# ISAE-PNX/SaDVIO

Measured on AMD Instinct MI355X. Metric: BA iterations/sec (ms/solve in ms_per_solve), 20-KF/8k-landmark window, higher is better.
Workload: dtype f64; 1 GPU; synthetic 20 KF x 8000 landmarks x 40000 reprojection factors (pixel), GN 10 iters (LM step attempts, early exits disabled); windows_per_gpu=1, parallelism=single window, n_kf=20, n_lmk=8000, n_obs=40000, reduced_dim=114

## Files before the change

sadvio_amd/csrc/ba_handle.h:

```cpp
#pragma once
#include <hip/hip_runtime.h>
#include <dlfcn.h>

#include <algorithm>
#include <chrono>
#include <cmath>
#include <cstdio>
#include <cstdlib>
#include <cstring>
#include <map>
#include <string>
#include <vector>

#include "../../include/sadvio_ba.h"
#include "kernels.h"
#include "layout_plan.h"
#include "dense_chol.h"
#include "marg_kernels.h"
#include "lm_kernels.h"
#include "long_kernels.h"
#include "viinit_kernels.h"
#include "nofov_kernels.h"

using namespace sadvio;
// ... 191 lines not shown
    ~CovBatchScratch() { if (pinned) (void)hipHostFree(pinned); }
};

struct RelScratch {
    DevBuf<int> pairs, kf_ptr, kf_lmk, n_shared, status;
    DevBuf<double> inf, Ak, Tab;
    std::vector<int> h_pairs, h_ptr, h_lmk, h_last;
    int csr_win = -1;
    int n_kf_lmk = 0;
};

struct EnvCfg {
    int debug = 0;
    int lm = -1, pf_wg = -1;
    int tile_rounds = 0, lm_subs = 0, band_c = 0;
    int cov_batch_lds = 1, cov_batch_scratch_mb = 1024;
    int cov_band = -1;
    int cov_sqrt = -1;
    int cov_cross_stage = -1;
    int long_min = 0;
    int long_min_env = 0;
    double jacobi_tol = 1e-14;
    bool marg_pivoted = false, marg_unpivoted = false, pchol_strict = false, no_lpt = false, no_pre = false, no_fork = false, no_bcr = false, imu_items = false, contig_tiles = false, c16_old_tail = false;
    void read() {
        auto on = [](const char* k) { return getenv(k) != nullptr; };
        auto num = [](const char* k, int unset) { const char* e = getenv(k); return e ? atoi(e) : unset; };
        debug = num("SADVIO_DEBUG", 0); lm = num("SADVIO_LM", -1); pf_wg = num("SADVIO_PF_WG", -1);
        tile_rounds = num("SADVIO_TILE_ROUNDS", 0); lm_subs = num("SADVIO_LM_SUBS", 0); band_c = num("SADVIO_BAND_C", 0);
        cov_batch_lds = num("SADVIO_COV_BATCH_LDS", 1); cov_batch_scratch_mb = num("SADVIO_COV_BATCH_SCRATCH_MB", 1024);
        cov_band = num("SADVIO_COV_BAND", -1); cov_sqrt = num("SADVIO_COV_SQRT", -1);
        cov_cross_stage = num("SADVIO_COV_CROSS_STAGE", -1);
        long_min_env = num("SADVIO_LONG_MIN", 0);
        if (long_min_env < 2 || long_min_env > MAX_LMK_OBS + 1) long_min_env = 0;
        if (const char* e = getenv("SADVIO_JACOBI_TOL")) jacobi_tol = atof(e);
        marg_pivoted = on("SADVIO_MARG_PIVOTED"); marg_unpivoted = on("SADVIO_MARG_UNPIVOTED"); pchol_strict = on("SADVIO_PCHOL_STRICT");
        no_lpt = on("SADVIO_NO_LPT"); no_pre = on("SADVIO_NO_PRE"); no_fork = on("SADVIO_NO_FORK");
        no_bcr = on("SADVIO_NO_BCR");
        contig_tiles = on("SADVIO_CONTIG_TILES");
        c16_old_tail = on("SADVIO_C16_OLD_TAIL");
        imu_items = on("SADVIO_IMU_ITEMS");
    }
};

struct sadvio_ba_handle {
    EnvCfg env;
    sadvio_ba_config cfg{};
    LayoutPlan plan;
    int device = 0;
    hipStream_t stream = nullptr;
    std::string err;
    std::vector<PriorDev> priors;
    std::vector<std::vector<PriorDev>> priors_per_win;
    std::vector<std::vector<ImuDev>> imus_per_win;
    std::vector<ImuDev> imus;
    DevBuf<int> d_big_info;
    DevBuf<double> d_big_M;
    DevBuf<double> d_big_Lx;
    DevBuf<double> d_big_linv;
    DevBuf<double> d_coll_band;
    DevBuf<double> d_bcr;
// ... 21 lines not shown
    DevBuf<LineDev> d_lines;
    DevBuf<LineObsDev> d_lobs;
    DevBuf<double> d_xline, d_line_scratch;
    int n_line_tot = 0, n_lobs_tot = 0;
    DevBuf<SparseDev> d_sparse;
    DevBuf<int> d_sp_list;
    int n_sp_list = 0;
    size_t n_sparse_tot = 0;
    DevBuf<double> d_sp_scratch;
    DevBuf<int> d_lmk_red, d_kept_obs, d_dp_ints;
    DevBuf<double> d_dp_data;
    int last_slots = 0;
    DevBuf<WinDev> d_win;
    DevBuf<Tile> d_tiles;
    DevBuf<double> d_kf_T0, d_xp, d_xv, d_xba, d_xbg, d_kf_vel, d_kf_ba, d_kf_bg;
    DevBuf<int> d_kf_fidx;
    DevBuf<double> d_cam_K, d_cam_T, d_cam_isig;
    DevBuf<double> d_lmk_p, d_xl, d_s_lmk;
    DevBuf<unsigned char> d_lmk_const;
    DevBuf<int> d_lmk_ob, d_lmk_oe, d_obs_kf, d_obs_cam, d_tile_kf, d_tile_row, d_tile_lmk;
    DevBuf<int> d_long_rec, d_long_kf, d_long_slot;
    DevBuf<int> d_pre_lane, d_pre_kf;
    bool pre_dirty = false;
    DevBuf<int> d_rank_col; DevBuf<double> d_rank_x;
    DevBuf<unsigned char> d_obs_slot, d_obs_lslot;
    DevBuf<int> d_chunk_ob, d_chunk_lm, d_tile_perm;
    DevBuf<int> d_jac_ints;
    DevBuf<double> d_jac_dbl;
    DevBuf<double> d_lm_hg, d_lm_dt, d_lm_sacc;
    DevBuf<int> d_lm_sub;
    int hidden_eig_count = 0;
    int marg_stats[4] = {0, 0, 0, 0};
    DevBuf<double> d_ptab;
    DevBuf<double> d_obs_meas;
    DevBuf<PriorDev> d_priors;
    DevBuf<double> d_prior_lin;
    DevBuf<ImuDev> d_imus;
    DevBuf<double> d_imu_scratch;
    DevBuf<double> d_S, d_gred, d_gfull, d_hdiag, d_delta, d_s_pose;
    DevBuf<LmState> d_states;
    DevBuf<double> d_trace;
    DevBuf<long long> d_tstart;
    DevBuf<IterAcc> d_acc;
    DevBuf<FinalRec> d_final;
    FinalRec* h_final = nullptr;
    double* h_deltas = nullptr; size_t h_deltas_cap = 0; bool deltas_cached = false;
// ... 70 lines not shown
```

sadvio_amd/csrc/ba_types.h:

```cpp
#pragma once
#include <stdint.h>

namespace sadvio {

struct SolveOpts {
    int max_num_iterations;
    int jacobi_scaling;
    int max_num_consecutive_invalid_steps;
    int pad;
    double function_tolerance, gradient_tolerance, parameter_tolerance;
    double initial_radius, max_radius, min_radius;
    double min_lm_diagonal, max_lm_diagonal, min_relative_decrease;
    double huber_a;
    double max_time_ticks;
};

struct WinDev {
    int n_kf, n_cam, n_lmk, n_obs;
    int kf_base, cam_base, lmk_base, obs_base;
    int n_free_kf, dpf, Np, Npose;
    long long S_off;
    int red_off;
    int tile_begin, tile_end;
    int prior_begin, prior_end;
// ... 7 lines not shown
    int kept_begin, kept_end;
    int sp_begin, sp_end;
    int spl_begin, spl_end;
    int line_begin, line_end;
    int lobs_begin, lobs_end;
};

struct Tile {
    int w;
    int lmk0, lmk1;
    int lmk_off;
    int n_lmk;
    int G;
    int kf_off, n_kf;
    int n_free;
    int lds_mode;
    int dpf, Np;
    int red_off;
    int cam_base, n_cam;
    int first_of_window;
    int kmax;
    int win_tile0, win_ntiles;
    int ld;
    long long S_off;
    int chunk0, chunk1;
};

struct PriorDev {
    int kf;
    int pad;
    double T_prior[12];
    double inf[6];
};

struct ImuDev {
    int kf_i, kf_j;
    double dt;
    double dR[9], dv[3], dp[3];
    double J_dR_bg[9], J_dv_ba[9], J_dv_bg[9], J_dp_ba[9], J_dp_bg[9];
    double W[81];
    double sa, sg;
    int win, pad;
};
struct SparseDev {
    int type, kf, lmk0, lmk1;
    int win, kf2;
// ... 51 lines not shown
    double lin_cost, fixed_cost, gmax;
    double cand_cost, mcc, step_norm2, cand_norm2;
    double pad;
};

constexpr int BUILD_THREADS = 256;
constexpr int BUILD_WAVES = BUILD_THREADS / 64;
constexpr int MAX_TILE_KF = 24;
constexpr int MAX_TILE_FREE_KF = 20;
constexpr int MAX_GEMM_FREE_KF = 5;
constexpr int MAX_WIN_CAM = 8;
constexpr int STAGE_VALS = 18;
constexpr int MAX_LMK_OBS = 64;
constexpr int MAX_LONG_OBS = 4096;
constexpr int MAX_LONG_KF = 512;
constexpr int LONG_THREADS = 256;
constexpr int LONG_REC = 6;
constexpr int SOLVE_THREADS = 512;
constexpr int SOLVE_KFC_STRIDE = 32;
constexpr int SOLVE_KFC = 32;
constexpr int PRIOR_LIN = 28;
constexpr int PRE_KF = 8;
constexpr int PRE_MAX_TILES = 1024;
constexpr int MAX_LDS_NP = 174;
constexpr int LM_CHUNK = 12;
constexpr int LM_PASS_THREADS = 64;

constexpr int c16_blocks(int n_rows) { return (n_rows + 15) >> 4; }
constexpr int c16_size(int N) { return (c16_blocks(N + 1) * (c16_blocks(N + 1) + 1) / 2) << 8; }

}
```

sadvio_amd/csrc/chol16.h:

```cpp
#pragma once
#include <hip/hip_runtime.h>

#include <type_traits>

#include "ba_types.h"


namespace sadvio {

typedef double c16_d4 __attribute__((ext_vector_type(4)));

constexpr int C16_STEP = 64;
constexpr int C16_PUB = 4 * C16_STEP;
constexpr int C16_WT = 16 * 17;
constexpr int C16_WORK = 2 * C16_PUB + 64 + C16_WT;

__host__ __device__ constexpr int c16_tile(int I, int J) { return ((I * (I + 1)) >> 1) + J; }
__host__ __device__ constexpr int c16_index(int i, int j) { return (c16_tile(i >> 4, j >> 4) << 8) + ((j & 15) << 4) + (i & 15); }

__device__ __forceinline__ double c16_readlane(double v, int lane) {
    int lo = __double2loint(v), hi = __double2hiint(v);
    lo = __builtin_amdgcn_readlane(lo, lane);
    hi = __builtin_amdgcn_readlane(hi, lane);
    return __hiloint2double(hi, lo);
}
__device__ __forceinline__ double c16_rsqrt(double d) {
    double y = __builtin_amdgcn_rsq(d);
    const double t = d * y;
    const double e = __builtin_fma(-t, y, 1.0);
    const double p = __builtin_fma(0.375, e, 0.5);
    const double q = e * p;
    return __builtin_fma(y, q, y);
}
__device__ __forceinline__ void c16_pair16(double v, double& e, double& o) {
    const unsigned lo = __double2loint(v), hi = __double2hiint(v);
    auto a = __builtin_amdgcn_permlane16_swap(lo, lo, false, false);
    auto b = __builtin_amdgcn_permlane16_swap(hi, hi, false, false);
    e = __hiloint2double(b[0], a[0]); o = __hiloint2double(b[1], a[1]);
}
__device__ __forceinline__ void c16_pair32(double v, double& l, double& u) {
    const unsigned lo = __double2loint(v), hi = __double2hiint(v);
// ... 404 lines not shown
```

sadvio_amd/csrc/kernels.h:

```cpp
#pragma once
#include "ba_types.h"
#include "device_math.h"
#include "chol16.h"

namespace sadvio {

struct DevPtrs {
    const WinDev* win;
    const Tile* tiles;
    const double* kf_T0;
    const int* kf_fidx;
    double* xp; double* xv; double* xba; double* xbg;
    long long xp_stride, xv_stride, xl_stride;
    const double* kf_vel; const double* kf_ba; const double* kf_bg;
    const double* cam_K; const double* cam_T; const double* cam_isig;
    const double* lmk_p; double* xl; double* s_lmk;
    const unsigned char* lmk_const;
    const int* lmk_ob; const int* lmk_oe;
    const int* obs_kf; const int* obs_cam; const double* obs_meas;
    const unsigned char* obs_slot;
    const int* tile_kf;
    const int* tile_lmk;
    const int* tile_row;
    const int4* pre_lane;
// ... 34 lines not shown
    const unsigned char* obs_lslot;
    double* lm_hg;
    double* lm_dt;
    long long lm_hg_stride, lm_dt_stride;
    const int* lm_sub;
    int lm_sub_per_item;
    int lm_ksub;
    double* lm_sacc;
    const LineDev* lines;
    const LineObsDev* lobs;
    double* xline;
    double* line_scratch;
    long long xline_stride;
    long long n_xp, n_xv, n_xl;
    int n_tiles;
    int state_stride;
    int n_win;
    long long* t_start;
    double* trace;
    long long* dbg_ts;
    int debug;
    int c16_old_tail;
    SolveOpts o;
};

#ifdef SADVIO_KERNEL_TS
#define SADVIO_TS(slot_, idx_) do { if ((P.debug & 4096) && blockIdx.x == 0 && threadIdx.x == 0 && slot == (slot_)) P.dbg_ts[idx_] = wall_clock64(); } while (0)
#define SADVIO_TS_PTR(cond_) ((cond_) ? P.dbg_ts : nullptr)
constexpr int DBG_WG_MAX = 1024, DBG_WG_BASE = 128, DBG_SLOTS = DBG_WG_BASE + 4 * DBG_WG_MAX;
#define SADVIO_WG_TS(slot_, which_) do { if ((P.debug & 4096) && blockIdx.x < DBG_WG_MAX && threadIdx.x == 0 && slot == (slot_)) { \
        P.dbg_ts[DBG_WG_BASE + 4 * blockIdx.x + (which_)] = wall_clock64(); \
        if ((which_) == 0) P.dbg_ts[DBG_WG_BASE + 4 * blockIdx.x + 3] = 0; \
        if ((which_) == 0) P.dbg_ts[DBG_WG_BASE + 4 * blockIdx.x + 2] = ((long long)__builtin_amdgcn_s_getreg(20 | (31 << 11)) << 32) | (unsigned)__builtin_amdgcn_s_getreg(4 | (31 << 11)); } } while (0)
#else
#define SADVIO_TS(slot_, idx_) do { } while (0)
#define SADVIO_TS_PTR(cond_) nullptr
#define SADVIO_WG_TS(slot_, which_) do { } while (0)
constexpr int DBG_SLOTS = 128;
#endif

__device__ __forceinline__ int tri(int i, int j) { return i * (i + 1) / 2 + j; }
__device__ __forceinline__ long long s_index(int ld, int i, int j) { return ld ? (long long)i * ld + j : (long long)c16_index(i, j); }

__device__ __forceinline__ void atomic_add_f64(double* p, double v) { unsafeAtomicAdd(p, v); }

__device__ __forceinline__ void atomic_max_u64(unsigned long long* p, unsigned long long v) { atomicMax(p, v); }
// ... 331 lines not shown
    return (b + 15) & ~(size_t)15;
}

__device__ __forceinline__ int tile_landmark(const Tile& T, const int* __restrict__ tile_lmk, int i) { return T.lmk_off >= 0 ? tile_lmk[T.lmk_off + i] : T.lmk0 + i; }

__global__ __launch_bounds__(BUILD_THREADS) void k_pre_packets(const Tile* __restrict__ tiles, const int* __restrict__ lmk_ob, const int* __restrict__ lmk_oe,
                                                               const int* __restrict__ tile_kf, const int* __restrict__ tile_lmk, const int* __restrict__ kf_fidx, int4* __restrict__ pre_lane,
                                                               int2* __restrict__ pre_kf) {
    const Tile T = tiles[blockIdx.x];
    const int tid = threadIdx.x;
    if (tid < BUILD_THREADS / 8) {
        const int lane0 = tid * 8, wv = lane0 >> 6, ln = lane0 & 63;
        const int G = T.G, lpw = 64 / G, grp = ln / G, q0 = ln - grp * G, nl = T.n_lmk;
        const bool valid = wv * lpw + grp < nl;
        const int gl = nl > 0 ? tile_landmark(T, tile_lmk, valid ? wv * lpw + grp : 0) : T.lmk0;
        const int ob = nl > 0 ? lmk_ob[gl] : 0, nobs = (valid && nl > 0) ? lmk_oe[gl] - ob : 0;
        pre_lane[(long long)blockIdx.x * (BUILD_THREADS / 8) + tid] = make_int4(gl, ob, nobs | (valid ? 1 << 16 : 0), q0);
    }
    if (tid < PRE_KF) {
        int2 e = make_int2(-1, -1);
        if (tid < T.n_kf) { e.x = tile_kf[T.kf_off + tid]; e.y = kf_fidx[e.x]; }
        pre_kf[(long long)blockIdx.x * PRE_KF + tid] = e;
    }
}

template <bool COST_ONLY> __device__ __forceinline__ void pose_factor_eval(const DevPtrs& P, int slot, int idx, int ln);
template <int FACTOR, bool RARE, bool IMU>
__global__ __launch_bounds__(BUILD_THREADS, IMU ? 1 : 2) void k_build(DevPtrs P, int slot, int max_tile_kf, int strip_doubles, int Rp) {
    extern __shared__ __attribute__((aligned(16))) char smem[];
    if (IMU && (int)blockIdx.x >= P.n_tiles) {
        pose_factor_eval<false>(P, slot, (int)blockIdx.x - P.n_tiles, threadIdx.x);
        return;
    }
    const Tile T = P.tiles[blockIdx.x];
    const int tid = threadIdx.x, wv = tid >> 6, ln = tid & 63;
    int4 pl = make_int4(0, -1, 0, 0);
    int2 pk = make_int2(-1, -1);
    if (P.pre_lane) {
        pl = P.pre_lane[(long long)blockIdx.x * (BUILD_THREADS / 8) + (tid >> 3)];
        pk = P.pre_kf[(long long)blockIdx.x * PRE_KF + tid / POSE_TAB];
    }
    SADVIO_TS(3, 32);
    SADVIO_WG_TS(3, 0);
    __shared__ double s_part[BUILD_WAVES * 4];
    double* poseTab = (double*)smem;
    double* camTab = poseTab + (size_t)max_tile_kf * POSE_TAB;
// ... 337 lines not shown
                    }
                }
            }
        }
        wave_lds_fence();
    }
        }
    if (gemm_mode && wv * lpw < nl) {
        const int lr = ln & 15, lk = ln >> 4;
        const int nt16 = (Nt + 15) >> 4;
#pragma unroll
        for (int pp = 0; pp < 3; pp++) {
            const int tr = pp < 1 ? 0 : 1, tc = pp - tr;
            if (tr < nt16) {
                const int col = 16 * tc + lr;
#pragma unroll
                for (int rg = 0; rg < 4; rg++) {
                    const int row = 16 * tr + lk + 4 * rg;
                    if (row < Nt && col <= row) atomic_add_f64(&Stile[tri(row, col)], -accs[pp][rg]);
                }
            }
        }
    }
    SADVIO_TS(3, 40);
    const double c = wave_sum(cost_part), f = wave_sum(fixed_part), gm = wave_max(gmax_part);
    if (ln == 0) { s_part[wv * 4] = c; s_part[wv * 4 + 1] = f; s_part[wv * 4 + 2] = gm; }
    __syncthreads();
    if (tid == 0) {
        double cs = 0.0, fs = 0.0, gs = 0.0;
        for (int k = 0; k < BUILD_WAVES; k++) { cs += s_part[k * 4]; fs += s_part[k * 4 + 1]; gs = fmax(gs, s_part[k * 4 + 2]); }
        TileAcc* ta = P.tacc + (long long)(slot & 1) * P.n_tiles + blockIdx.x;
        ta->lin_cost = cs; ta->fixed_cost = fs; ta->gmax = gs;
    }
    SADVIO_TS(3, 41);
    if (lds_mode) {
        int* growTab = (int*)stage;
        for (int k = tid; k < T.n_kf; k += blockDim.x) {
            const int r = rowTab[k];
            if (r >= 0) {
                const int fi = P.kf_fidx[P.tile_kf[T.kf_off + k]];
#pragma unroll
                for (int i = 0; i < 6; i++) growTab[r + i] = fi * dpf + i;
            }
        }
        __syncthreads();
        if (T.ld) {
            for (int row = wv; row < Nt; row += BUILD_WAVES) {
                const long long grow = (long long)growTab[row] * T.ld;
                const double* srow = Stile + tri(row, 0);
                for (int col = ln; col <= row; col += 64) {
                    const double v = srow[col];
                    if (v != 0.0) atomic_add_f64(&Sg[grow + growTab[col]], v);
                }
            }
        } else {
            for (int col = wv; col < Nt; col += BUILD_WAVES) {
                const int gc = growTab[col];
                for (int row = col + ln; row < Nt; row += 64) {
// ... 2243 lines not shown
```

sadvio_amd/csrc/layout_driver.h:

```cpp
#pragma once
#include "ba_handle.h"

namespace {

__global__ void k_dense_prior_prepare(const double* J, double* Jt, int nf, int n) {
    const long long idx = (long long)blockIdx.x * blockDim.x + threadIdx.x;
    if (idx < (long long)nf * n) {
        const int i = (int)(idx / n), a = (int)(idx - (long long)i * n);
        Jt[(size_t)a * nf + i] = J[idx];
    }
}

__global__ void k_sym_from_lower(const double* __restrict__ A, int n, double* __restrict__ H) {
    const long long idx = (long long)blockIdx.x * blockDim.x + threadIdx.x;
    if (idx >= (long long)n * n) return;
    const int i = (int)(idx / n), j = (int)(idx - (long long)i * n);
    H[idx] = i >= j ? A[idx] : A[(size_t)j * n + i];
}

LayoutIn layout_inputs(sadvio_ba_handle* h) {
    LayoutIn in;
    in.src = &h->src; in.sparse_per_win = &h->sparse_per_win; in.dprior_per_win = &h->dprior_per_win; in.lines_per_win = &h->lines_per_win;
    in.prior_valid = h->prior.valid; in.prior_serial = h->prior.serial; in.prior_n_full = h->prior.n_full; in.prior_n = h->prior.n;
    in.world = h->world; in.has_coll = h->coll_fn != nullptr;
    in.tile_rounds = h->env.tile_rounds; in.lm = h->env.lm; in.lm_subs = h->env.lm_subs;
    in.contig_tiles = h->env.contig_tiles; in.no_lpt = h->env.no_lpt; in.no_pre = h->env.no_pre;
    in.long_min = h->env.long_min;
    return in;
}

template <typename T>
void queue_table(sadvio_ba_handle* h, DevBuf<T>& dst, const std::vector<T>& src) { h->up.add(dst.p, src.data(), src.size() * sizeof(T)); }

int layout_reduced_device(sadvio_ba_handle* h) {
    LayoutPlan& P = h->plan;
    const long long s_b = P.s_tot, nrb = P.n_rank_b;
    const int red_b = P.np_tot;
    HIP_TRY(h->d_S.alloc((size_t)std::max<long long>(P.red_total, 1)));
    h->d_gred.set_view(h->d_S.p + s_b, (size_t)red_b); h->d_gfull.set_view(h->d_gred.p + red_b, (size_t)red_b);
    h->d_hdiag.set_view(h->d_gfull.p + red_b, (size_t)red_b); h->d_rank_b.set_view(h->d_hdiag.p + red_b, (size_t)nrb);
    HIP_TRY(h->d_rank_s.alloc((size_t)nrb));
    HIP_TRY(h->d_delta.alloc((size_t)std::max(red_b, 1))); HIP_TRY(h->d_s_pose.alloc((size_t)std::max(red_b, 1)));
    HIP_TRY(hipMemsetAsync(h->d_S.p, 0, sizeof(double) * (size_t)std::max<long long>(P.red_total, 1), h->stream));
    HIP_TRY(hipMemsetAsync(h->d_rank_s.p, 0, sizeof(double) * (size_t)nrb, h->stream));
    HIP_TRY(h->d_sparse.alloc(std::max<size_t>(P.sparse.size(), 1))); HIP_TRY(h->d_sp_scratch.alloc(2 * std::max<size_t>(P.sparse.size(), 1) * SPARSE_J));
    HIP_TRY(h->d_sp_list.alloc(std::max<size_t>(P.sp_list.size(), 1)));
    h->n_sparse_tot = P.sparse.size(); h->n_sp_list = (int)P.sp_list.size();
    h->n_line_tot = (int)P.lines.size(); h->n_lobs_tot = (int)P.lobs.size();
    HIP_TRY(h->d_lines.alloc(std::max<size_t>(P.lines.size(), 1))); HIP_TRY(h->d_lobs.alloc(std::max<size_t>(P.lobs.size(), 1)));
    HIP_TRY(h->d_xline.alloc(std::max<size_t>(12 * P.lines.size(), 1))); HIP_TRY(h->d_line_scratch.alloc(std::max<size_t>(P.lobs.size(), 1) * LINE_ROW));
    HIP_TRY(h->d_tiles.alloc(P.tiles.size())); HIP_TRY(h->d_lmk_red.alloc(P.lmk_red.size())); HIP_TRY(h->d_lmk_const.alloc(P.lmk_const_red.size()));
    HIP_TRY(h->d_kept_obs.alloc(P.kept.size())); HIP_TRY(h->d_dp_ints.alloc(P.dp_ints.size())); HIP_TRY(h->d_dp_data.alloc((size_t)std::max<long long>(P.dp_total, 1)));
    queue_table(h, h->d_sparse, P.sparse); queue_table(h, h->d_sp_list, P.sp_list); queue_table(h, h->d_lines, P.lines); queue_table(h, h->d_lobs, P.lobs);
    queue_table(h, h->d_tiles, P.tiles); queue_table(h, h->d_lmk_red, P.lmk_red); queue_table(h, h->d_lmk_const, P.lmk_const_red);
    queue_table(h, h->d_kept_obs, P.kept); queue_table(h, h->d_dp_ints, P.dp_ints);
    if (!P.preps.empty()) HIP_TRY(hipMemsetAsync(h->d_dp_data.p, 0, sizeof(double) * (size_t)P.dp_total, h->stream));
    for (const DensePrep& pr : P.preps) {
        const DensePriorHost& D = h->dprior_per_win[pr.w];
        double* J = h->d_dp_data.p + pr.off;
        double* r0 = J + 2 * (size_t)pr.nf * pr.n + (size_t)pr.n * pr.n;
        if (D.resident) {
            HIP_TRY(hipMemcpyAsync(J, h->prior.J.p, sizeof(double) * (size_t)pr.nf * pr.n, hipMemcpyDeviceToDevice, h->stream));
            HIP_TRY(hipMemcpyAsync(r0, h->prior.r0.p, sizeof(double) * (size_t)pr.nf, hipMemcpyDeviceToDevice, h->stream));
        } else {
            h->up.add(J, D.J.data(), sizeof(double) * (size_t)pr.nf * pr.n);
            h->up.add(r0, D.r0.data(), sizeof(double) * (size_t)pr.nf);
        }
    }
    if (!P.preps.empty()) HIP_TRY(h->up.flush(h->stream));
    for (const DensePrep& pr : P.preps) {
        double* J = h->d_dp_data.p + pr.off;
        double* Jt = J + (size_t)pr.nf * pr.n;
        double* H = Jt + (size_t)pr.n * pr.nf;
        const long long items = (long long)pr.nf * pr.n;
        hipLaunchKernelGGL(k_dense_prior_prepare, dim3((unsigned)((items + 255) / 256)), dim3(256), 0, h->stream, J, Jt, pr.nf, pr.n);
        if (h->dprior_per_win[pr.w].resident && h->prior.hg_valid && h->prior.n == pr.n)
            hipLaunchKernelGGL(k_sym_from_lower, dim3((unsigned)(((long long)pr.n * pr.n + 255) / 256)), dim3(256), 0, h->stream, h->prior.H.p, pr.n, H);
        else
// ... 26 lines not shown
    }
    HIP_TRY(h->d_priors.alloc(h->priors.size()));
    HIP_TRY(h->d_prior_lin.alloc(2 * h->priors.size() * (size_t)PRIOR_LIN));
    if (!h->priors.empty())
        h->up.add(h->d_priors.p, h->priors.data(), h->priors.size() * sizeof(PriorDev));
    h->imus.clear();
    for (size_t w = 0; w < wins.size(); w++) {
        wins[w].d.imu_begin = (int)h->imus.size();
        for (auto& f : h->imus_per_win[w]) { h->imus.push_back(f); h->imus.back().win = (int)w; }
        wins[w].d.imu_end = (int)h->imus.size();
    }
    HIP_TRY(h->d_imus.alloc(h->imus.size()));
    HIP_TRY(h->d_imu_scratch.alloc(2 * h->imus.size() * (size_t)IMU_ROW));
    if (!h->imus.empty())
        h->up.add(h->d_imus.p, h->imus.data(), h->imus.size() * sizeof(ImuDev));
    std::vector<WinDev> wd(wins.size());
    for (size_t w = 0; w < wins.size(); w++) wd[w] = wins[w].d;
    h->up.add(h->d_win.p, wd.data(), wd.size() * sizeof(WinDev));
    HIP_TRY(h->up.flush(h->stream));
    if (h->plan.pre_ok && h->pre_dirty) {
        hipLaunchKernelGGL(k_pre_packets, dim3((unsigned)h->plan.tiles.size()), dim3(BUILD_THREADS), 0, h->stream, h->d_tiles.p, h->d_lmk_ob.p, h->d_lmk_oe.p, h->d_tile_kf.p,
                           h->d_tile_lmk.p, h->d_kf_fidx.p, (int4*)h->d_pre_lane.p, (int2*)h->d_pre_kf.p);
        h->pre_dirty = false;
    }
    return SADVIO_OK;
}

int layout_build(sadvio_ba_handle* h) {
    const bool dbg_t = (h->env.debug & 8192) != 0;
    auto t_start = std::chrono::steady_clock::now();
    auto lap = [&](const char* what) { if (dbg_t) { auto t = std::chrono::steady_clock::now(); fprintf(stderr, "[sadvio dbg] build_layout %-14s %.3f ms\n", what, std::chrono::duration<double, std::milli>(t - t_start).count()); t_start = t; } };
    HIP_TRY(hipSetDevice(h->device));
    h->uploaded = false; h->solved = false;
    h->up.reset();
    LayoutPlan& P = h->plan;
    int rc = layout_plan(layout_inputs(h), P, h->err, lap);
    if (rc != SADVIO_OK) return rc;
    const size_t kf_b = P.n_kf_tot, lmk_b = std::max(P.n_lmk_tot, 1), n_tiles = P.tiles.size();
    if (h->env.debug) {
        auto chunks = [&](int ti) { return P.tiles[ti].chunk1 - P.tiles[ti].chunk0; };
        if (P.want_lm && n_tiles)
            fprintf(stderr, "[sadvio dbg] chunks per tile: largest %d, median %d, smallest %d\n", chunks(P.perm.front()), chunks(P.perm[n_tiles / 2]), chunks(P.perm.back()));
        int hist[32] = {0}, modes[3] = {0};
        for (auto& t : P.tiles) { hist[std::min(t.n_free, 31)]++; modes[t.lds_mode]++; }
        fprintf(stderr, "[sadvio dbg] %zu tiles, modes global/atomic/gemm = %d/%d/%d, max_tile_kf %d, n_free histogram:", n_tiles, modes[0], modes[1], modes[2], P.max_tile_kf);
        for (int i = 0; i < 32; i++) if (hist[i]) fprintf(stderr, " %d:%d", i, hist[i]);
// ... 17 lines not shown
    HIP_TRY(h->d_xba.alloc(2 * 3 * kf_b)); HIP_TRY(h->d_xbg.alloc(2 * 3 * kf_b));
    HIP_TRY(h->d_kf_vel.alloc(P.kf_vel.size())); HIP_TRY(h->d_kf_ba.alloc(P.kf_ba.size())); HIP_TRY(h->d_kf_bg.alloc(P.kf_bg.size()));
    HIP_TRY(h->d_cam_K.alloc(P.cam_K.size())); HIP_TRY(h->d_cam_T.alloc(P.cam_T.size())); HIP_TRY(h->d_cam_isig.alloc(P.cam_isig.size()));
    HIP_TRY(h->d_lmk_p.alloc(P.lmk_p.size())); HIP_TRY(h->d_xl.alloc(2 * 3 * lmk_b));
    HIP_TRY(h->d_s_lmk.alloc(3 * lmk_b));
    HIP_TRY(h->d_lmk_ob.alloc(P.lmk_ob.size())); HIP_TRY(h->d_lmk_oe.alloc(P.lmk_oe.size()));
    HIP_TRY(h->d_obs_kf.alloc(P.obs_kf.size())); HIP_TRY(h->d_obs_cam.alloc(P.obs_cam.size())); HIP_TRY(h->d_obs_meas.alloc(P.obs_meas.size()));
    queue_table(h, h->d_chunk_ob, P.chunk_ob); queue_table(h, h->d_chunk_lm, P.chunk_lm); queue_table(h, h->d_obs_lslot, P.obs_lslot);
    queue_table(h, h->d_tile_perm, P.perm); queue_table(h, h->d_lm_sub, P.sub);
    queue_table(h, h->d_kf_T0, P.kf_T0); queue_table(h, h->d_kf_fidx, P.kf_fidx); queue_table(h, h->d_kf_vel, P.kf_vel);
    queue_table(h, h->d_kf_ba, P.kf_ba); queue_table(h, h->d_kf_bg, P.kf_bg); queue_table(h, h->d_cam_K, P.cam_K); queue_table(h, h->d_cam_T, P.cam_T);
    queue_table(h, h->d_cam_isig, P.cam_isig); queue_table(h, h->d_lmk_p, P.lmk_p);
    queue_table(h, h->d_lmk_ob, P.lmk_ob); queue_table(h, h->d_lmk_oe, P.lmk_oe); queue_table(h, h->d_obs_kf, P.obs_kf);
    queue_table(h, h->d_obs_cam, P.obs_cam); queue_table(h, h->d_obs_meas, P.obs_meas); queue_table(h, h->d_tile_kf, P.tile_kf);
    queue_table(h, h->d_tile_row, P.tile_row); queue_table(h, h->d_tile_lmk, P.tile_lmk); queue_table(h, h->d_obs_slot, P.obs_slot);
    if (P.n_long > 0) {
        HIP_TRY(h->d_long_rec.alloc(P.long_rec.size())); HIP_TRY(h->d_long_kf.alloc(P.long_kf.size())); HIP_TRY(h->d_long_slot.alloc(P.long_slot.size()));
        queue_table(h, h->d_long_rec, P.long_rec); queue_table(h, h->d_long_kf, P.long_kf); queue_table(h, h->d_long_slot, P.long_slot);
    }
    if (P.pre_ok) {
        HIP_TRY(h->d_pre_lane.alloc((size_t)4 * (BUILD_THREADS / 8) * n_tiles)); HIP_TRY(h->d_pre_kf.alloc((size_t)2 * PRE_KF * n_tiles));
        h->pre_dirty = true;
    }
    h->rel.csr_win = -1;
    lap("alloc+queue");
    rc = layout_reduced_device(h);
    if (rc != SADVIO_OK) return rc;
    lap("reduced device");
    rc = upload_priors(h);
    if (rc != SADVIO_OK) return rc;
    lap("flush");
    h->uploaded = true;
    for (auto& k : h->kclasses) { k.total_ms = 0; k.launches = 0; }
    return SADVIO_OK;
}

}
```

sadvio_amd/csrc/layout_plan.h:

```cpp
#pragma once
#include <algorithm>
#include <cstdint>
#include <cstring>
#include <string>
#include <vector>

#include "../../include/sadvio_ba.h"
#include "ba_types.h"
#include "tile_pack.h"

namespace sadvio {

struct SrcWin {
    sadvio_flat_window v{};
    std::vector<int64_t> kf_id, lmk_id;
    std::vector<double> kf_T, kf_vel, kf_ba, kf_bg, cam_K, cam_T, cam_sigma, lmk_p, obs_meas;
    std::vector<uint8_t> kf_const, lmk_const;
    std::vector<int32_t> lmk_obs_ptr, obs_kf, obs_cam;
    std::vector<int32_t> a_ptr, a_kf, a_cam, a_src;
    std::vector<double> a_meas;
    std::vector<double> u_cam_K, u_cam_T, u_cam_sigma;
    std::vector<int32_t> u_obs_cam;
    std::vector<int> cam_map;
};
// ... 20 lines not shown
    std::vector<int> ptr, obs_kf, obs_cam;
    int n() const { return (int)id.size(); }
};

struct LayoutScratch {
    std::vector<int> pack_order, pack_cut, pkf, run_max, mark, add, kfs, slot_of;
    std::vector<int> rem, rem_ptr, rem_kf, rem_run;
    std::vector<long long> long_key;
    std::vector<char> held;
};

struct LayoutIn {
    std::vector<SrcWin>* src = nullptr;
    const std::vector<std::vector<sadvio_sparse_prior>>* sparse_per_win = nullptr;
    const std::vector<DensePriorHost>* dprior_per_win = nullptr;
    const std::vector<LineSetHost>* lines_per_win = nullptr;
    bool prior_valid = false;
    unsigned long long prior_serial = 0;
    int prior_n_full = 0, prior_n = 0;
    int world = 1;
    bool has_coll = false;
    int tile_rounds = 0, lm = -1, lm_subs = 0;
    bool contig_tiles = false, no_lpt = false, no_pre = false;
    int long_min = 0;
};

struct DensePrep { long long off; int nf, n, w; };

struct LayoutPlan {
    std::vector<sadvio_flat_window> views;
    std::vector<std::vector<char>> sp_elim;
    std::vector<int> n_obs_user;
    std::vector<HostWin> wins;
    int factor_type = 0;
    int n_kf_tot = 0, n_cam_tot = 0, n_lmk_tot = 0, n_obs_tot = 0;
    int max_n_kf = 0, max_npose = 0;
    bool user_lmk_const = false;
    std::vector<int> long_rec, long_kf, long_slot;
    std::vector<char> is_long;
    int n_long = 0, long_max_kf = 0;
    std::vector<double> kf_T0, kf_vel, kf_ba, kf_bg, cam_K, cam_T, cam_isig, lmk_p, obs_meas;
    std::vector<int> kf_fidx, lmk_ob, lmk_oe, obs_kf, obs_cam;
    std::vector<unsigned char> lmk_const;
    std::vector<int> obs_perm;
    std::vector<Tile> tiles;
    std::vector<int> tile_kf, tile_row, tile_lmk;
    std::vector<unsigned char> obs_slot;
    int max_tile_kf = 1, max_tile_free = 0, max_gemm_free = 0;
    bool gemm_run4 = false;
    std::vector<int> chunk_ob, chunk_lm, perm, sub;
    std::vector<unsigned char> obs_lslot;
    bool want_lm = false;
    bool lm_ok = false;
    long long lm_landmarks = 0;
    int lm_sub_obs = 0;
    int lm_ksub = 1, lm_max_cam = 1, lm_n_sub = 0;
    int lm_sub_per_item = 8;
    bool pre_ok = false;
    std::vector<int> lmk_red, kept, dp_ints, sp_list;
    std::vector<unsigned char> lmk_const_red;
    std::vector<SparseDev> sparse;
    std::vector<LineDev> lines;
    std::vector<LineObsDev> lobs;
    std::vector<DensePrep> preps;
    long long dp_total = 0;
    long long s_tot = 0, red_total = 0, n_rank_b = 0;
    int np_tot = 0, n_kept = 0, max_np = 0, n_big = 0;
    bool has_lmk_const = false;
    LayoutScratch ls;
};

inline int check_flat_window(const sadvio_flat_window& F, int w, std::string& err) {
    if (F.n_kf <= 0 || F.n_cam < 0 || F.n_lmk < 0 || F.n_obs < 0 || !F.kf_T_f_w || (F.n_cam > 0 && (!F.cam_K || !F.cam_T_s_f)) ||
        (F.n_obs > 0 && F.n_cam == 0) ||
        (F.n_lmk > 0 && (!F.lmk_p || !F.lmk_obs_ptr)) || (F.n_obs > 0 && (!F.obs_kf || !F.obs_cam || !F.obs_meas))) {
        err = "set_windows: missing array in window " + std::to_string(w);
        return SADVIO_E_INVALID_ARG;
    }
    if (F.n_lmk > 0 && (F.lmk_obs_ptr[0] != 0 || F.lmk_obs_ptr[F.n_lmk] != F.n_obs)) {
        err = "set_windows: lmk_obs_ptr is not a CSR over n_obs";
        return SADVIO_E_INVALID_ARG;
// ... 451 lines not shown
    }
    auto& perm = P.perm;
    perm.resize(P.tiles.size());
    for (size_t i = 0; i < perm.size(); i++) perm[i] = (int)i;
    if (want_lm && !in.no_lpt)
        std::stable_sort(perm.begin(), perm.end(), [&](int a, int b) {
            return P.tiles[a].chunk1 - P.tiles[a].chunk0 > P.tiles[b].chunk1 - P.tiles[b].chunk0; });
    P.sub.clear();
    if (in.lm_subs > 0) P.lm_sub_per_item = in.lm_subs;
    if (want_lm)
        for (int ti : perm) {
            const Tile& t = P.tiles[ti];
            for (int q = 0, l0 = t.lmk0; l0 < t.lmk1; l0 += LM_PASS_THREADS * P.lm_sub_per_item, q += P.lm_sub_per_item) { P.sub.push_back(ti); P.sub.push_back(q); }
        }
    P.lm_n_sub = (int)P.sub.size() / 2;
    if (P.tile_kf.empty()) { P.tile_kf.push_back(0); P.tile_row.push_back(-1); }
    if (P.tile_lmk.empty()) P.tile_lmk.push_back(0);
    if (P.long_rec.empty()) P.long_rec.assign(LONG_REC, 0);
    if (P.long_kf.empty()) P.long_kf.push_back(0);
    if (P.long_slot.empty()) P.long_slot.push_back(0);
    P.pre_ok = !P.tiles.empty() && P.tiles.size() <= PRE_MAX_TILES && !in.no_pre;
}

inline int layout_reduced_plan(const LayoutIn& in, LayoutPlan& P, std::string& err) {
    const int n_windows = (int)P.wins.size();
    const auto& dpriors = *in.dprior_per_win;
    for (int w = 0; w < n_windows && w < (int)dpriors.size(); w++) {
        const DensePriorHost& D = dpriors[w];
        if (D.n_full > 0 && D.resident && (!in.prior_valid || in.prior_serial != D.serial || in.prior_n_full != D.n_full || in.prior_n != D.n)) {
            err = "the handle's prior changed after set_dense_prior(SADVIO_PRIOR_RESIDENT) attached it to a window: attach it again"; return SADVIO_E_STATE;
        }
    }
    if (P.n_long > 0)
        for (int w = 0; w < n_windows && w < (int)dpriors.size(); w++) {
            const int lb = P.wins[w].d.lmk_base;
            const DensePriorHost& D = dpriors[w];
            bool bad = false;
            for (size_t i = 0; i < D.lmk_index.size(); i++) bad |= D.n_full > 0 && D.lmk_col[i] >= 0 && P.is_long[lb + D.lmk_index[i]];
            for (const sadvio_sparse_prior& sp : (*in.sparse_per_win)[w]) {
                if (sp.type != SADVIO_SPARSE_IMU_PRIOR && sp.type != SADVIO_SPARSE_RELATIVE_POSE) bad |= P.is_long[lb + sp.lmk0] != 0;
                if (sp.type == SADVIO_SPARSE_LMK_TO_LMK) bad |= P.is_long[lb + sp.lmk1] != 0;
            }
            if (bad) { err = "long tracks: a prior factor keeps or touches a landmark on the long path"; return SADVIO_E_INVALID_ARG; }
        }
    int red_b = 0; long long s_b = 0;
    P.max_np = 0; P.n_big = 0;
// ... 100 lines not shown
                    memcpy(q.meas, &LS.meas[(size_t)ms * ob], sizeof(double) * ms);
                    lobs.push_back(q);
                }
                lines.push_back(o);
            }
        }
        d.line_end = (int)lines.size(); d.lobs_end = (int)lobs.size();
        d.ld = d.Np > MAX_LDS_NP ? d.Np : 0;
        d.S_off = s_b; d.red_off = red_b;
        red_b += d.Np; s_b += d.ld ? (((long long)d.Np * d.Np + 1) & ~1LL) : (long long)c16_size(d.Np);
        if (d.ld) P.n_big++; else P.max_np = std::max(P.max_np, d.Np);
        for (int ti = d.tile_begin; ti < d.tile_end; ti++) {
            Tile& t = P.tiles[ti];
            t.Np = d.Np; t.red_off = d.red_off; t.S_off = d.S_off; t.ld = d.ld;
        }
    }
    P.np_tot = red_b; P.s_tot = s_b; P.dp_total = dp_total;
    P.n_kept = (int)kept.size() / 3;
    P.has_lmk_const = P.user_lmk_const || any_red;
    P.n_rank_b = (long long)n_windows * in.world * 4;
    P.red_total = s_b + 3LL * red_b + P.n_rank_b;
    if (kept.empty()) kept.assign(3, 0);
    if (dp_ints.empty()) dp_ints.push_back(0);
    return SADVIO_OK;
}

template <typename Lap>
inline int layout_plan(const LayoutIn& in, LayoutPlan& P, std::string& err, Lap&& lap) {
    const int n_windows = (int)in.src->size();
    layout_views(in, P);
    lap("views");
    for (int w = 0; w < n_windows; w++) {
        const sadvio_flat_window& F = P.views[w];
        if (F.factor_type != P.views[0].factor_type || (F.factor_type != SADVIO_FACTOR_PIXEL && F.factor_type != SADVIO_FACTOR_ANGULAR)) {
            err = "set_windows: all windows of a batch must share one factor_type";
            return SADVIO_E_INVALID_ARG;
        }
    }
    layout_windows(n_windows, P.views.data(), P);
    if (const int rc = layout_long(in, P, err)) return rc;
    lap("  validate");
    layout_concat_begin(P);
    for (int w = 0; w < n_windows; w++) {
        layout_concat(P, w);
        lap("  concat");
        int rc = layout_sort(in, P, w, err);
        if (rc != SADVIO_OK) return rc;
        rc = layout_long_lists(P, w, err);
        if (rc != SADVIO_OK) return rc;
        lap("  sort+permute");
        rc = layout_tiles(in, P, w, err);
        if (rc != SADVIO_OK) return rc;
    }
    lap("concat+tiles");
    layout_chunks(in, P);
    lap("chunks");
    const int rc = layout_reduced_plan(in, P, err);
    lap("layout_reduced");
    return rc;
}

}
```

sadvio_amd/csrc/solve_driver.h:

```cpp
#pragma once
#include <cstddef>
#include <type_traits>

#include "ba_handle.h"

namespace {

DevPtrs make_ptrs(sadvio_ba_handle* h, const SolveOpts& o, int state_stride) {
    DevPtrs P{};
    P.win = h->d_win.p; P.tiles = h->d_tiles.p;
    P.kf_T0 = h->d_kf_T0.p; P.kf_fidx = h->d_kf_fidx.p;
    P.xp = h->d_xp.p; P.xv = h->d_xv.p; P.xba = h->d_xba.p; P.xbg = h->d_xbg.p;
    P.xp_stride = 6LL * h->plan.n_kf_tot; P.xv_stride = 3LL * h->plan.n_kf_tot; P.xl_stride = 3LL * h->plan.n_lmk_tot;
    P.kf_vel = h->d_kf_vel.p; P.kf_ba = h->d_kf_ba.p; P.kf_bg = h->d_kf_bg.p;
    P.cam_K = h->d_cam_K.p; P.cam_T = h->d_cam_T.p; P.cam_isig = h->d_cam_isig.p;
    P.lmk_p = h->d_lmk_p.p; P.xl = h->d_xl.p; P.s_lmk = h->d_s_lmk.p;
    P.lmk_const = h->plan.has_lmk_const ? h->d_lmk_const.p : nullptr;
    P.lmk_ob = h->d_lmk_ob.p; P.lmk_oe = h->d_lmk_oe.p;
    P.obs_kf = h->d_obs_kf.p; P.obs_cam = h->d_obs_cam.p; P.obs_meas = h->d_obs_meas.p;
    P.obs_slot = h->d_obs_slot.p; P.tile_kf = h->d_tile_kf.p; P.tile_lmk = h->d_tile_lmk.p; P.tile_row = h->d_tile_row.p;
    P.pre_lane = h->plan.pre_ok ? (const int4*)h->d_pre_lane.p : nullptr; P.pre_kf = h->plan.pre_ok ? (const int2*)h->d_pre_kf.p : nullptr;
    P.ptab = h->d_ptab.p; P.ptab_stride = (long long)POSE_TAB * h->plan.n_kf_tot;
    P.priors = h->d_priors.p; P.prior_lin = h->d_prior_lin.p; P.prior_lin_stride = (long long)h->priors.size() * PRIOR_LIN; P.n_prior_tot = (int)h->priors.size();
    P.imus = h->d_imus.p; P.imu_scratch = h->d_imu_scratch.p; P.imu_scratch_stride = (long long)h->imus.size() * IMU_ROW;
    P.S = h->d_S.p; P.gred = h->d_gred.p; P.gfull = h->d_gfull.p; P.hdiag = h->d_hdiag.p;
    P.delta = h->d_delta.p; P.s_pose = h->d_s_pose.p;
    P.dbg_ts = h->d_dbg.p;
    P.trace = h->d_trace.p; P.t_start = h->d_tstart.p;
    P.states = h->d_states.p; P.acc = h->d_acc.p; P.tacc = h->d_tacc.p; P.n_tiles = (int)h->plan.tiles.size();
    P.state_stride = state_stride;
    P.final_out = h->h_final ? h->h_final : h->d_final.p;
    P.big_info = h->d_big_info.p;
    P.world = h->world; P.rank = h->rank; P.rank_b = h->d_rank_b.p; P.rank_s = h->d_rank_s.p;
    P.lmk_red = h->d_lmk_red.p; P.kept_obs = h->d_kept_obs.p; P.n_kept = h->plan.n_kept;
    P.dp_data = h->d_dp_data.p; P.dp_ints = h->d_dp_ints.p;
    P.sparse = h->d_sparse.p; P.sp_scratch = h->d_sp_scratch.p; P.sp_list = h->d_sp_list.p;
    P.sp_scratch_stride = (long long)std::max<size_t>(h->n_sparse_tot, 1) * SPARSE_J; P.n_imu_tot = (int)h->imus.size(); P.n_sp_list = h->n_sp_list;
    P.chunk_ob = h->d_chunk_ob.p; P.chunk_lm = h->d_chunk_lm.p; P.tile_perm = h->d_tile_perm.p; P.obs_lslot = h->d_obs_lslot.p;
    P.lm_hg = h->d_lm_hg.p; P.lm_hg_stride = (long long)LM_HG * std::max(h->plan.n_lmk_tot, 1);
    P.lm_dt = h->d_lm_dt.p; P.lm_dt_stride = (long long)LM_DT * std::max<long long>((long long)h->plan.tiles.size(), 1) * h->plan.lm_ksub;
    P.lm_sub = h->d_lm_sub.p; P.lm_ksub = h->plan.lm_ksub; P.lm_sub_per_item = h->plan.lm_sub_per_item; P.lm_sacc = h->plan.lm_ok ? h->d_lm_sacc.p : nullptr;
    P.lines = h->d_lines.p; P.lobs = h->d_lobs.p; P.xline = h->d_xline.p; P.line_scratch = h->d_line_scratch.p;
    P.xline_stride = 6LL * h->n_line_tot;
    P.n_xp = (long long)h->d_xp.n; P.n_xv = (long long)h->d_xv.n; P.n_xl = (long long)h->d_xl.n;
// ... 500 lines not shown
```

Baseline: 19660 BA iterations/s.

## Precompute per-tile flush index map for LDS Schur tile accumulation

Adds a per-tile precomputed map from local packed-triangle entries to global reduced-matrix offsets (dense or c16-packed), built once on device after layout. The LDS-mode flush in the build kernel then reads prefetched index pairs and issues atomics directly, instead of recomputing global row tables and index arithmetic every iteration. This spends extra device memory, bounded by a budget, and extra global reads of the map in exchange for less per-iteration index work.

```diff
diff --git a/sadvio_amd/csrc/ba_handle.h b/sadvio_amd/csrc/ba_handle.h
--- a/sadvio_amd/csrc/ba_handle.h
+++ b/sadvio_amd/csrc/ba_handle.h
@@ -237,6 +237,8 @@
     int long_min_env = 0;
     double jacobi_tol = 1e-14;
     bool marg_pivoted = false, marg_unpivoted = false, pchol_strict = false, no_lpt = false, no_pre = false, no_fork = false, no_bcr = false, imu_items = false, contig_tiles = false, c16_old_tail = false;
+    bool no_flush_map = false;
+    int flush_budget = -1;
     void read() {
         auto on = [](const char* k) { return getenv(k) != nullptr; };
         auto num = [](const char* k, int unset) { const char* e = getenv(k); return e ? atoi(e) : unset; };
@@ -251,6 +253,7 @@
         marg_pivoted = on("SADVIO_MARG_PIVOTED"); marg_unpivoted = on("SADVIO_MARG_UNPIVOTED"); pchol_strict = on("SADVIO_PCHOL_STRICT");
         no_lpt = on("SADVIO_NO_LPT"); no_pre = on("SADVIO_NO_PRE"); no_fork = on("SADVIO_NO_FORK");
         no_bcr = on("SADVIO_NO_BCR");
+        no_flush_map = on("SADVIO_NO_FLUSH_MAP"); flush_budget = num("SADVIO_FLUSH_MAP_BUDGET", -1);
         contig_tiles = on("SADVIO_CONTIG_TILES");
         c16_old_tail = on("SADVIO_C16_OLD_TAIL");
         imu_items = on("SADVIO_IMU_ITEMS");
@@ -318,6 +321,8 @@
     DevBuf<int> d_long_rec, d_long_kf, d_long_slot;
     DevBuf<int> d_pre_lane, d_pre_kf;
     bool pre_dirty = false;
+    DevBuf<int> d_tile_grow, d_tile_grow_off, d_flush_map;
+    bool flush_dirty = false;
     DevBuf<int> d_rank_col; DevBuf<double> d_rank_x;
     DevBuf<unsigned char> d_obs_slot, d_obs_lslot;
     DevBuf<int> d_chunk_ob, d_chunk_lm, d_tile_perm;
diff --git a/sadvio_amd/csrc/ba_types.h b/sadvio_amd/csrc/ba_types.h
--- a/sadvio_amd/csrc/ba_types.h
+++ b/sadvio_amd/csrc/ba_types.h
@@ -53,6 +53,7 @@
     int kmax;
     int win_tile0, win_ntiles;
     int ld;
+    int flush_base;
     long long S_off;
     int chunk0, chunk1;
 };
@@ -150,11 +151,16 @@
 constexpr int PRIOR_LIN = 28;
 constexpr int PRE_KF = 8;
 constexpr int PRE_MAX_TILES = 1024;
+constexpr int FLUSH_MAP_BUDGET = 1 << 22;
 constexpr int MAX_LDS_NP = 174;
 constexpr int LM_CHUNK = 12;
 constexpr int LM_PASS_THREADS = 64;
 
 constexpr int c16_blocks(int n_rows) { return (n_rows + 15) >> 4; }
 constexpr int c16_size(int N) { return (c16_blocks(N + 1) * (c16_blocks(N + 1) + 1) / 2) << 8; }
+constexpr int c16_tile(int I, int J) { return ((I * (I + 1)) >> 1) + J; }
+constexpr int c16_index(int i, int j) { return (c16_tile(i >> 4, j >> 4) << 8) + ((j & 15) << 4) + (i & 15); }
+
+constexpr int flush_offset(int ld, int grow_row, int grow_col) { return ld ? grow_row * ld + grow_col : c16_index(grow_row, grow_col); }
 
 }
diff --git a/sadvio_amd/csrc/chol16.h b/sadvio_amd/csrc/chol16.h
--- a/sadvio_amd/csrc/chol16.h
+++ b/sadvio_amd/csrc/chol16.h
@@ -15,8 +15,6 @@
 constexpr int C16_WT = 16 * 17;
 constexpr int C16_WORK = 2 * C16_PUB + 64 + C16_WT;
 
-__host__ __device__ constexpr int c16_tile(int I, int J) { return ((I * (I + 1)) >> 1) + J; }
-__host__ __device__ constexpr int c16_index(int i, int j) { return (c16_tile(i >> 4, j >> 4) << 8) + ((j & 15) << 4) + (i & 15); }
 
 __device__ __forceinline__ double c16_readlane(double v, int lane) {
     int lo = __double2loint(v), hi = __double2hiint(v);
diff --git a/sadvio_amd/csrc/kernels.h b/sadvio_amd/csrc/kernels.h
--- a/sadvio_amd/csrc/kernels.h
+++ b/sadvio_amd/csrc/kernels.h
@@ -80,6 +80,7 @@
     int debug;
     int c16_old_tail;
     SolveOpts o;
+    const int* flush_map;
 };
 
 #ifdef SADVIO_KERNEL_TS
@@ -457,6 +458,24 @@
         if (tid < T.n_kf) { e.x = tile_kf[T.kf_off + tid]; e.y = kf_fidx[e.x]; }
         pre_kf[(long long)blockIdx.x * PRE_KF + tid] = e;
     }
+}
+
+__global__ __launch_bounds__(BUILD_THREADS) void k_pre_flush(const Tile* __restrict__ tiles, const int* __restrict__ grow_off, const int* __restrict__ tile_grow,
+                                                             int* __restrict__ flush_map) {
+    const Tile T = tiles[blockIdx.x];
+    const int go = grow_off[blockIdx.x];
+    if (T.flush_base < 0 || go < 0) return;
+    const int Nt = 6 * T.n_free, tri_n = Nt * (Nt + 1) / 2;
+    const int* grow = tile_grow + go;
+    int2* pairs = (int2*)(flush_map + T.flush_base);
+    for (int r = threadIdx.x >> 5; r < Nt; r += BUILD_THREADS >> 5) {
+        const int gr = grow[r];
+        for (int c = threadIdx.x & 31; c <= r; c += 32) {
+            const int at = T.ld ? r * (r + 1) / 2 + c : c * Nt - c * (c - 1) / 2 + (r - c);
+            pairs[at] = make_int2(r * (r + 1) / 2 + c, flush_offset(T.ld, gr, grow[c]));
+        }
+    }
+    for (int i = threadIdx.x; i < Nt; i += BUILD_THREADS) flush_map[T.flush_base + 2 * tri_n + i] = grow[i];
 }
 
 template <bool COST_ONLY> __device__ __forceinline__ void pose_factor_eval(const DevPtrs& P, int slot, int idx, int ln);
@@ -840,6 +859,14 @@
             }
         }
     }
+    const int2* fmap = (P.flush_map != nullptr && T.flush_base >= 0) ? (const int2*)(P.flush_map + T.flush_base) : nullptr;
+    int2 fm0 = make_int2(0, 0), fm1 = make_int2(0, 0);
+    int frow = 0;
+    if (fmap) {
+        if (tid < tri_n) fm0 = fmap[tid];
+        if (tid + BUILD_THREADS < tri_n) fm1 = fmap[tid + BUILD_THREADS];
+        if (tid < Nt) frow = ((const int*)(fmap + tri_n))[tid];
+    }
     SADVIO_TS(3, 40);
     const double c = wave_sum(cost_part), f = wave_sum(fixed_part), gm = wave_max(gmax_part);
     if (ln == 0) { s_part[wv * 4] = c; s_part[wv * 4 + 1] = f; s_part[wv * 4 + 2] = gm; }
@@ -851,7 +878,25 @@
         ta->lin_cost = cs; ta->fixed_cost = fs; ta->gmax = gs;
     }
     SADVIO_TS(3, 41);
-    if (lds_mode) {
+    if (lds_mode && fmap) {
+        if (tid < tri_n) { const double v = Stile[fm0.x]; if (v != 0.0) atomic_add_f64(&Sg[fm0.y], v); }
+        if (tid + BUILD_THREADS < tri_n) { const double v = Stile[fm1.x]; if (v != 0.0) atomic_add_f64(&Sg[fm1.y], v); }
+        for (int e0 = tid + 2 * BUILD_THREADS; e0 < tri_n; e0 += 4 * BUILD_THREADS) {
+            int2 m[4];
+#pragma unroll
+            for (int u = 0; u < 4; u++) { const int e = e0 + u * BUILD_THREADS; m[u] = e < tri_n ? fmap[e] : make_int2(0, 0); }
+#pragma unroll
+            for (int u = 0; u < 4; u++) {
+                const int e = e0 + u * BUILD_THREADS;
+                if (e < tri_n) { const double v = Stile[m[u].x]; if (v != 0.0) atomic_add_f64(&Sg[m[u].y], v); }
+            }
+        }
+        if (tid < Nt) {
+            if (gT[tid] != 0.0) atomic_add_f64(&gredg[frow], gT[tid]);
+            if (gfT[tid] != 0.0) atomic_add_f64(&gfullg[frow], gfT[tid]);
+            if (hdT[tid] != 0.0) atomic_add_f64(&hdg[frow], hdT[tid]);
+        }
+    } else if (lds_mode) {
         int* growTab = (int*)stage;
         for (int k = tid; k < T.n_kf; k += blockDim.x) {
             const int r = rowTab[k];
diff --git a/sadvio_amd/csrc/layout_driver.h b/sadvio_amd/csrc/layout_driver.h
--- a/sadvio_amd/csrc/layout_driver.h
+++ b/sadvio_amd/csrc/layout_driver.h
@@ -26,6 +26,7 @@
     in.tile_rounds = h->env.tile_rounds; in.lm = h->env.lm; in.lm_subs = h->env.lm_subs;
     in.contig_tiles = h->env.contig_tiles; in.no_lpt = h->env.no_lpt; in.no_pre = h->env.no_pre;
     in.long_min = h->env.long_min;
+    in.no_flush_map = h->env.no_flush_map; in.flush_budget = h->env.flush_budget;
     return in;
 }
 
@@ -54,6 +55,9 @@
     queue_table(h, h->d_sparse, P.sparse); queue_table(h, h->d_sp_list, P.sp_list); queue_table(h, h->d_lines, P.lines); queue_table(h, h->d_lobs, P.lobs);
     queue_table(h, h->d_tiles, P.tiles); queue_table(h, h->d_lmk_red, P.lmk_red); queue_table(h, h->d_lmk_const, P.lmk_const_red);
     queue_table(h, h->d_kept_obs, P.kept); queue_table(h, h->d_dp_ints, P.dp_ints);
+    HIP_TRY(h->d_flush_map.alloc((size_t)std::max<long long>(P.flush_total, 1)));
+    h->flush_dirty = P.flush_total > 0;
+    if (h->env.debug) fprintf(stderr, "[sadvio dbg] flush map: %lld ints\n", P.flush_total);
     if (!P.preps.empty()) HIP_TRY(hipMemsetAsync(h->d_dp_data.p, 0, sizeof(double) * (size_t)P.dp_total, h->stream));
     for (const DensePrep& pr : P.preps) {
         const DensePriorHost& D = h->dprior_per_win[pr.w];
@@ -126,6 +130,10 @@
         hipLaunchKernelGGL(k_pre_packets, dim3((unsigned)h->plan.tiles.size()), dim3(BUILD_THREADS), 0, h->stream, h->d_tiles.p, h->d_lmk_ob.p, h->d_lmk_oe.p, h->d_tile_kf.p,
                            h->d_tile_lmk.p, h->d_kf_fidx.p, (int4*)h->d_pre_lane.p, (int2*)h->d_pre_kf.p);
         h->pre_dirty = false;
+    }
+    if (h->flush_dirty) {
+        hipLaunchKernelGGL(k_pre_flush, dim3((unsigned)h->plan.tiles.size()), dim3(BUILD_THREADS), 0, h->stream, h->d_tiles.p, h->d_tile_grow_off.p, h->d_tile_grow.p, h->d_flush_map.p);
+        h->flush_dirty = false;
     }
     return SADVIO_OK;
 }
@@ -189,6 +197,8 @@
         HIP_TRY(h->d_pre_lane.alloc((size_t)4 * (BUILD_THREADS / 8) * n_tiles)); HIP_TRY(h->d_pre_kf.alloc((size_t)2 * PRE_KF * n_tiles));
         h->pre_dirty = true;
     }
+    HIP_TRY(h->d_tile_grow.alloc(P.tile_grow.size())); HIP_TRY(h->d_tile_grow_off.alloc(P.tile_grow_off.size()));
+    queue_table(h, h->d_tile_grow, P.tile_grow); queue_table(h, h->d_tile_grow_off, P.tile_grow_off);
     h->rel.csr_win = -1;
     lap("alloc+queue");
     rc = layout_reduced_device(h);
diff --git a/sadvio_amd/csrc/layout_plan.h b/sadvio_amd/csrc/layout_plan.h
--- a/sadvio_amd/csrc/layout_plan.h
+++ b/sadvio_amd/csrc/layout_plan.h
@@ -66,6 +66,8 @@
     bool has_coll = false;
     int tile_rounds = 0, lm = -1, lm_subs = 0;
     bool contig_tiles = false, no_lpt = false, no_pre = false;
+    bool no_flush_map = false;
+    int flush_budget = -1;
     int long_min = 0;
 };
 
@@ -101,6 +103,9 @@
     int lm_ksub = 1, lm_max_cam = 1, lm_n_sub = 0;
     int lm_sub_per_item = 8;
     bool pre_ok = false;
+    std::vector<int> tile_grow;
+    std::vector<int> tile_grow_off;
+    long long flush_total = 0;
     std::vector<int> lmk_red, kept, dp_ints, sp_list;
     std::vector<unsigned char> lmk_const_red;
     std::vector<SparseDev> sparse;
@@ -598,6 +603,47 @@
     P.pre_ok = !P.tiles.empty() && P.tiles.size() <= PRE_MAX_TILES && !in.no_pre;
 }
 
+inline void layout_flush_rows(const LayoutIn& in, LayoutPlan& P) {
+    P.tile_grow.clear();
+    P.tile_grow_off.assign(std::max<size_t>(P.tiles.size(), 1), -1);
+    for (size_t ti = 0; ti < P.tiles.size(); ti++) {
+        Tile& t = P.tiles[ti];
+        t.flush_base = -1;
+        if (in.no_flush_map || t.lds_mode == 0) continue;
+        P.tile_grow_off[ti] = (int)P.tile_grow.size();
+        for (int k = 0; k < t.n_kf; k++) {
+            if (P.tile_row[t.kf_off + k] < 0) continue;
+            const int fi = P.kf_fidx[P.tile_kf[t.kf_off + k]];
+            for (int i = 0; i < 6; i++) P.tile_grow.push_back(fi * t.dpf + i);
+        }
+    }
+    if (P.tile_grow.empty()) P.tile_grow.push_back(0);
+}
+
+constexpr long long flush_map_ints(int n_free) { return 6LL * n_free * (6LL * n_free + 1) + 6LL * n_free; }
+
+inline void layout_flush_map(const LayoutIn& in, LayoutPlan& P) {
+    static_assert(c16_size(MAX_LDS_NP) > 0, "offsets into the tile-packed image are ints");
+    const long long budget = in.flush_budget >= 0 ? in.flush_budget : FLUSH_MAP_BUDGET;
+    long long total = 0;
+    bool fits = !in.no_flush_map;
+    for (size_t ti = 0; ti < P.tiles.size(); ti++) {
+        const Tile& t = P.tiles[ti];
+        if (P.tile_grow_off[ti] < 0) continue;
+        total += flush_map_ints(t.n_free);
+        if (t.ld && (long long)t.Np * t.ld > 0x7fffffffLL) fits = false;
+    }
+    if (total > budget || total > 0x7fffffffLL) fits = false;
+    P.flush_total = 0;
+    for (size_t ti = 0; ti < P.tiles.size(); ti++) {
+        Tile& t = P.tiles[ti];
+        t.flush_base = -1;
+        if (!fits || P.tile_grow_off[ti] < 0) continue;
+        t.flush_base = (int)P.flush_total;
+        P.flush_total += flush_map_ints(t.n_free);
+    }
+}
+
 inline int layout_reduced_plan(const LayoutIn& in, LayoutPlan& P, std::string& err) {
     const int n_windows = (int)P.wins.size();
     const auto& dpriors = *in.dprior_per_win;
@@ -744,6 +790,7 @@
     P.red_total = s_b + 3LL * red_b + P.n_rank_b;
     if (kept.empty()) kept.assign(3, 0);
     if (dp_ints.empty()) dp_ints.push_back(0);
+    layout_flush_map(in, P);
     return SADVIO_OK;
 }
 
@@ -776,6 +823,7 @@
     }
     lap("concat+tiles");
     layout_chunks(in, P);
+    layout_flush_rows(in, P);
     lap("chunks");
     const int rc = layout_reduced_plan(in, P, err);
     lap("layout_reduced");
diff --git a/sadvio_amd/csrc/solve_driver.h b/sadvio_amd/csrc/solve_driver.h
--- a/sadvio_amd/csrc/solve_driver.h
+++ b/sadvio_amd/csrc/solve_driver.h
@@ -20,6 +20,7 @@
     P.obs_kf = h->d_obs_kf.p; P.obs_cam = h->d_obs_cam.p; P.obs_meas = h->d_obs_meas.p;
     P.obs_slot = h->d_obs_slot.p; P.tile_kf = h->d_tile_kf.p; P.tile_lmk = h->d_tile_lmk.p; P.tile_row = h->d_tile_row.p;
     P.pre_lane = h->plan.pre_ok ? (const int4*)h->d_pre_lane.p : nullptr; P.pre_kf = h->plan.pre_ok ? (const int2*)h->d_pre_kf.p : nullptr;
+    P.flush_map = h->plan.flush_total > 0 ? h->d_flush_map.p : nullptr;
     P.ptab = h->d_ptab.p; P.ptab_stride = (long long)POSE_TAB * h->plan.n_kf_tot;
     P.priors = h->d_priors.p; P.prior_lin = h->d_prior_lin.p; P.prior_lin_stride = (long long)h->priors.size() * PRIOR_LIN; P.n_prior_tot = (int)h->priors.size();
     P.imus = h->d_imus.p; P.imu_scratch = h->d_imu_scratch.p; P.imu_scratch_stride = (long long)h->imus.size() * IMU_ROW;
```

Result: no change. 19650 BA iterations/s (-0.1%).
